# Sachin-A/TraceWeaver

Hardware: AMD Instinct MI355X
Metric: spans/sec reconstructed + assignment accuracy vs ground truth (higher is better)
Workload: dtype int64 timestamps, f64 scores; 1 GPU; media_microservices shape (6 services, E in {1,1,1,1,2,4}), 100000 requests/service x 16 replicas per GPU, concurrency 1.6, two-pass reconstruction, device mixture refit; spans_per_gpu=25600000, spans_total=25600000, parallelism=units sharded, 1 rank(s), backend none

## Files before the change

traceweaver_amd/csrc/tw_device.h:

```cpp
#pragma once
#include <hip/hip_runtime.h>
#include <stdint.h>

#include "traceweaver_amd.h"

namespace tw {

constexpr int kMaxEp = TW_MAX_EP;
constexpr int kTopK = TW_TOPK;
constexpr int kMaxComp = TW_MAX_COMP;
constexpr int kMaxWin = TW_MAX_WINDOW;
constexpr int kCandWords = TW_CAND_WORDS;
constexpr int kEnumStretches = 8;
constexpr int kTile = 128;
constexpr int kCoop = 256;
constexpr int32_t kNoOwner = 0x7f7f7f7f;

struct UnitDev {
    int64_t in_off;
    int64_t ie_off;
    int64_t ep_off[kMaxEp + 1];
    int32_t n_in;
    int32_t E;
    int32_t nblk;
// ... 31 lines not shown

struct Dev {
    const UnitDev* units;
    const TileDev* tiles;
    int32_t n_units, n_tiles;
    int32_t tile_spans;
    int64_t n_in_total, n_out_total;
    int32_t batch_size, batch_mis;
    const int64_t *in_start, *in_end, *out_start, *out_end;
    int64_t *in_end_sorted, *out_end_sorted;
    double* gparam;
    const int32_t* mix_n;
    const double* mix_c;
    int64_t* pm_val;
    int32_t* pm_idx;
    uint8_t* pc;
    int32_t* seg;
    uint8_t* win_end;
    int32_t* wid;
    int32_t* w_last;
    int32_t* unit_nwin;
    uint8_t* w_dirty;
    int32_t* w_conf;
    int32_t* unit_ndirty;
    int32_t* tk_n;
    int64_t* leaves;
    int64_t* leaves0;
    int32_t* chosen;
    uint8_t* rep;
    int32_t* tkr_n;
    int32_t *tk_idx, *tkr_idx;
    double *tk_score, *tkr_score;
    int32_t* c_lo;
    int32_t* c_hi;
    uint64_t* c_bits;
    uint64_t* gone;
    uint8_t* gone_valid;
    int64_t* leaves_r;
    unsigned long long* frontier_big;
    int32_t* frontier_big_busy;
    int32_t frontier_big_slots;
    int32_t* frontier_busy;
    unsigned long long* frontier;
    int32_t* round_changed;
    int32_t* parent;
    int32_t* owner;
    double* gaps;
    const int64_t* gs_off;
    int64_t* unit_stats;
    int32_t* heavy_count;
    int32_t* heavy_next;
    int32_t *heavy_unit, *heavy_win;
    int32_t *tiny_unit, *tiny_win;
    int32_t *rheavy_unit, *rheavy_win, *rtiny_unit, *rtiny_win;
    int32_t *hard_unit, *hard_win;
    int32_t* heavy_in_count;
    int32_t* heavy_in_next;
    int32_t heavy_in_off[kMaxEp + 2];
    int32_t* enum_snap;
    int32_t* enum_stretch_next;
    int32_t *heavy_in_unit, *heavy_in_idx;
    int32_t* heavy_big_count;
    int32_t *heavy_big_unit, *heavy_big_idx;
    int32_t heavy_big_off[kMaxEp + 2];
    int32_t* heavy_big_part;
    int32_t* heavy_big_slot;
    int32_t part_off[kMaxEp + 2];
    int32_t split_twins;
    int32_t* part_used;
    int32_t defer_min_e;
    int32_t defer_cap;
    unsigned long long* defer_list;
    int32_t* defer_used;
    int32_t* defer_count;
    int32_t *part_lo, *part_hi;
    int32_t* part_lvl;
    int32_t* any_wide;
    int32_t* redo_count;
    int32_t* defer_refused;
    int32_t lean_min_e;
    int32_t tile_max_deep;
    int32_t lean_grid;
    int32_t tile_rank;
    double* pair_pool;
    int32_t* pair_busy;
    int32_t* fb_count;
    int32_t* fb_total;
    int32_t *fb_unit, *fb_idx, *fb_part, *fb_slot;
    int32_t* split_count;
    int32_t *split_unit, *split_idx, *split_slot, *split_parts;
    int32_t* part_n;
    int64_t* part_leaves;
    double* part_score;
    int32_t* part_idx;
    unsigned long long* part_bits;
    int32_t* part_logn;
    double* part_log_sc;
    unsigned long long* part_log_ix;
    int32_t* err;
    unsigned long long* prof;
};

__device__ __forceinline__ int32_t hi_word(double x) { return (int32_t)(__double_as_longlong(x) >> 32); }
__device__ __forceinline__ uint32_t lo_word(double x) { return (uint32_t)__double_as_longlong(x); }
__device__ __forceinline__ double with_hi(double x, int32_t hi) {
    return __longlong_as_double((long long)(((uint64_t)(uint32_t)hi << 32) | (uint64_t)lo_word(x)));
}
__device__ __forceinline__ double dnan() { return __longlong_as_double(0x7ff8000000000000LL); }
__device__ __forceinline__ double dinf() { return __longlong_as_double(0x7ff0000000000000LL); }

__device__ inline double tw_log(double x) {
    const double ln2_hi = 6.93147180369123816490e-01, ln2_lo = 1.90821492927058770002e-10,
                 two54 = 1.80143985094819840000e+16, Lg1 = 6.666666666666735130e-01,
                 Lg2 = 3.999999999940941908e-01, Lg3 = 2.857142874366239149e-01,
                 Lg4 = 2.222219843214978396e-01, Lg5 = 1.818357216161805012e-01,
                 Lg6 = 1.531383769920937332e-01, Lg7 = 1.479819860511658591e-01;
    int32_t k = 0, hx = hi_word(x);
    if (hx < 0x00100000) {
        if (((hx & 0x7fffffff) | lo_word(x)) == 0) return -dinf();
        if (hx < 0) return dnan();
        k -= 54;
        x *= two54;
        hx = hi_word(x);
    }
    if (hx >= 0x7ff00000) return x + x;
    k += (hx >> 20) - 1023;
    hx &= 0x000fffff;
    int32_t i = (hx + 0x95f64) & 0x100000;
    x = with_hi(x, hx | (i ^ 0x3ff00000));
    k += (i >> 20);
    double f = x - 1.0, dk = (double)k;
    if ((0x000fffff & (2 + hx)) < 3) {
        if (f == 0.0) return k == 0 ? 0.0 : dk * ln2_hi + dk * ln2_lo;
        double R = f * f * (0.5 - 0.33333333333333333 * f);
        return k == 0 ? f - R : dk * ln2_hi - ((R - dk * ln2_lo) - f);
    }
    double s = f / (2.0 + f), z = s * s, w = z * z;
    i = hx - 0x6147a;
    int32_t j = 0x6b851 - hx;
    double t1 = w * (Lg2 + w * (Lg4 + w * Lg6));
    double t2 = z * (Lg1 + w * (Lg3 + w * (Lg5 + w * Lg7)));
    double R = t2 + t1;
    if ((i | j) > 0) {
        double hfsq = 0.5 * f * f;
        return k == 0 ? f - (hfsq - s * (hfsq + R)) : dk * ln2_hi - ((hfsq - (s * (hfsq + R) + dk * ln2_lo)) - f);
    }
    return k == 0 ? f - s * (f - R) : dk * ln2_hi - ((s * (f - R) - dk * ln2_lo) - f);
}

__device__ inline double tw_exp(double x) {
    const double o_threshold = 7.09782712893383973096e+02, u_threshold = -7.45133219101941108420e+02,
                 ln2HI = 6.93147180369123816490e-01, ln2LO = 1.90821492927058770002e-10,
                 invln2 = 1.44269504088896338700e+00, P1 = 1.66666666666666019037e-01,
                 P2 = -2.77777777770155933842e-03, P3 = 6.61375632143793436117e-05,
                 P4 = -1.65339022054652515390e-06, P5 = 4.13813679705723846039e-08,
                 twom1000 = 9.33263618503218878990e-302;
    double hi = 0.0, lo = 0.0;
    int32_t k = 0, hx = hi_word(x);
    const int32_t xsb = (hx >> 31) & 1;
    hx &= 0x7fffffff;
    if (hx >= 0x40862E42) {
        if (hx >= 0x7ff00000) {
            if (((hx & 0xfffff) | lo_word(x)) != 0) return x + x;
            return xsb == 0 ? x : 0.0;
        }
        if (x > o_threshold) return dinf();
// ... 139 lines not shown
```

traceweaver_amd/csrc/tw_engine.hip:

```cpp
#include <algorithm>
#include <chrono>
#include <cmath>
#include <cstdio>
#include <cstdlib>
#include <cstring>
#include <functional>
#include <string>
#include <type_traits>
#include <vector>

#include <hip/hip_runtime.h>
#include <rocprim/rocprim.hpp>

#include "traceweaver_amd.h"
#include "tw_kernels.h"
#include "tw_fit.h"
#include "tw_eval.h"
#include "tw_skip.h"
#include "tw_load.h"
#include "tw_baselines.h"
#include "tw_stitch.h"
#include "tw_attr.h"
#include "tw_conf.h"
#include "tw_dist.h"
#include "tw_sig.h"
#include "tw_prof.h"
#include "tw_order.h"

using namespace tw;

namespace {

constexpr int kMaxRepairRounds = 1 << 20;
enum { ST_EMPTY = 0, ST_LOADED = 1, ST_PASS1 = 2, ST_MIX = 3, ST_PASS2 = 4 };
enum { EV_BEGIN = 0, EV_PARAMS, EV_ENUM0, EV_ENUM1, EV_WIN, EV_SEL, EV_REPAIR, EV_END, EV_COUNT };
enum { SE_STITCH = 0, SE_ATTR = 5, SE_CONF = 9, SE_DIST = 13, SE_SIG = 18, SE_PROF = 22, SE_COUNT = 26 };

int env_int(const char* name, int dflt) {
    const char* v = getenv(name);
    return (v && *v) ? atoi(v) : dflt;
}

struct Mt19937 {
    uint32_t mt[624];
    int idx = 624;
    explicit Mt19937(uint32_t seed = 0u) {
        mt[0] = seed;
        for (int i = 1; i < 624; i++) mt[i] = 1812433253u * (mt[i - 1] ^ (mt[i - 1] >> 30)) + (uint32_t)i;
    }
    uint32_t next() {
        if (idx >= 624) {
            for (int i = 0; i < 624; i++) {
                const uint32_t y = (mt[i] & 0x80000000u) | (mt[(i + 1) % 624] & 0x7fffffffu);
                mt[i] = mt[(i + 397) % 624] ^ (y >> 1) ^ ((y & 1u) ? 0x9908b0dfu : 0u);
            }
            idx = 0;
        }
        uint32_t y = mt[idx++];
        y ^= y >> 11;
        y ^= (y << 7) & 0x9d2c5680u;
        y ^= (y << 15) & 0xefc60000u;
        y ^= y >> 18;
        return y;
    }
    double random_sample() {
        const uint32_t a = next() >> 5, b = next() >> 6;
        return ((double)a * 67108864.0 + (double)b) / 9007199254740992.0;
    }
};

}

struct tw_engine {
    int device = 0;
    hipStream_t stream = nullptr;
    hipStream_t cls_stream[kMaxEp + 1] = {};
    hipEvent_t cls_ev[kMaxEp + 2] = {};
    hipStream_t sel_stream[3] = {};
    hipStream_t sel_stream2[3] = {};
    int64_t select_fork_min = 0;
    hipEvent_t prep_ev = nullptr;
    hipEvent_t post_fork[kMaxEp + 1] = {}, post_join[kMaxEp + 1][3] = {}, post_done[kMaxEp + 1] = {};
    hipEvent_t tile_ev[kMaxEp + 1] = {};
    hipStream_t cls_stream2[kMaxEp + 1] = {};
    hipEvent_t stretch_ev[kMaxEp + 1][kEnumStretches] = {}, stretch_done[kMaxEp + 1] = {};
    int enum_stretches = 1, stretch_min_tiles = 2048;
    int heavy_grid = 4096, select_grid = 0;
    int debug_lists = 0;
    int32_t first_lists[3][kMaxEp + 1] = {};
    hipEvent_t gate_ev = nullptr;
    int tile_gate = 0;
    int stage_min_tiles = 1024;
    int32_t *rank_in = nullptr, *rank_out = nullptr;
    bool class_params = false;
    int prio_min_e = 0, prio_high = 0;
    bool prio_any = false;
    int pipeline = 1;
    std::string err;
    int state = ST_EMPTY;
    int tile = kTile;
    int tile_threads = 2;
    int tile_single = 1;
    int tile_rank = 1;
    int block_params = 1;
    int tile_single_threads = 1;
    int tile_pair = 1;
    int tile_pair_threads = 2;
    int coop = kCoop;
    std::vector<UnitDev> units;
    std::vector<TileDev> tiles;
    std::vector<int64_t> gs_off_h;
    std::vector<void*> allocs;
    void* arena = nullptr;
    size_t arena_cap = 0;
    bool arena_open = false;
    std::vector<std::pair<std::function<void(void*)>, size_t>> arena_req;
    Dev P{};
    int64_t n_ie = 0, n_gp = 0, n_slots = 0, n_gaps = 0;
    PairVI* agg_pair = nullptr;
    int32_t *agg_i32 = nullptr, *agg_i32b = nullptr;
    uint32_t *seg_in = nullptr, *seg_out = nullptr;
    int n_seg_out = 0;
    void* sort_tmp = nullptr;
    size_t sort_tmp_bytes = 0;
    double* mix_p_dev = nullptr;
    int32_t* mix_n_dev = nullptr;
    double* mix_c_dev = nullptr;
    double* gaps_sorted = nullptr;
    double* fit_models = nullptr;
    double* fit_uval = nullptr;
    int32_t *fit_ustart = nullptr, *fit_row_n = nullptr, *fit_row_uniq = nullptr;
    double* fit_centres = nullptr;
    double *fit_tape = nullptr, *fit_tape100 = nullptr;
    int64_t* fit_tape_off = nullptr;
    int64_t fit_tape_cap = 0;
    bool fit_runs_pending = false;
    bool fit_prepared = false;
    int tile_sub_max = 8;
    int32_t hard_pass1[kMaxEp + 1] = {};
    int8_t wide_pass1[kMaxEp + 1] = {};
    int32_t split_pass1[kMaxEp + 1] = {};
    int lean_pool = 512;
    bool pass1_done = false;
    std::vector<int32_t> fit_max_n;
    bool fit_max_n_valid = false;
    Mt19937 fit_rng;
    uint32_t fit_seed = 0;
    int32_t* slot_unit = nullptr;
    int32_t* tile_ids = nullptr;
    int32_t* ctr = nullptr;
    int64_t ctr_round_ints = 0, ctr_pass_ints = 0;
    int32_t tile_cls_off[kMaxEp + 2] = {};
    BlockRef* blk_tab = nullptr;
    int32_t blk_cls_off[kMaxEp + 2] = {};
    uint32_t *seg_gap = nullptr, *seg_gap_end = nullptr, *seg_gap_dst = nullptr;
    unsigned long long *comp_a = nullptr, *comp_b = nullptr;
    int64_t comp_cap = 0, n_gap_scored = 0;
    int32_t *truth = nullptr, *in_trace = nullptr;
    uint8_t* trace_bad = nullptr;
    unsigned long long* eval_counts = nullptr;
    int64_t n_traces = 0, trace_cap = 0;
    uint8_t* slot_scored = nullptr;
    int64_t n_gap_rows = 0;
    unsigned long long* key_acc = nullptr;
    double fit_ms = 0.0;
    int rounds = 0;
    bool skip_mode = false;
    SkipUnitDev* skip_units = nullptr;
    int32_t* skip_perm = nullptr; int64_t* skip_tw = nullptr; int32_t* skip_pool = nullptr; double* skip_dist = nullptr; long long* skip_fetch = nullptr;
    int64_t skip_fetch_n = 0;
    int64_t *orig_is = nullptr, *orig_ie = nullptr, *orig_os = nullptr, *orig_oe = nullptr;
    int32_t *orig_truth = nullptr, *orig_trace = nullptr;
    bool scaled_upload = false;
    hipEvent_t ev[EV_COUNT] = {};
    double ms[6] = {0, 0, 0, 0, 0, 0};
    StitchDev S{};
    int32_t* given_parent = nullptr;
    bool rows_set = false, parents_given = false, stitched = false;
    int64_t rows_cap = 0, st_trees = 0;
    int stitched_pass = -1;
    bool stitched_truth = false;
    AttrDev A{};
    bool groups_set = false, attributed = false;
    int64_t groups_cap = 0, attr_rows_cap = 0;
    ConfDev C{};
    int64_t conf_rows_cap = 0;
// ... 694 lines not shown
    int32_t* d_rank = trace_rank != nullptr ? (int32_t*)scratch(4 * n_in) : nullptr;
    unsigned long long *ka = (unsigned long long*)scratch(8 * n_max), *kb = (unsigned long long*)scratch(8 * n_max);
    uint32_t *perm = (uint32_t*)scratch(4 * n_max), *perm_alt = (uint32_t*)scratch(4 * n_max);
    uint32_t* perm_in = (uint32_t*)scratch(4 * n_in);
    int32_t *pos_in = (int32_t*)scratch(4 * n_in), *pos_out = (int32_t*)scratch(4 * n_out);
    if (!L.x || !L.xe || !L.y || !L.ye || !L.rank_in || !L.rank_out || !L.row_in || !L.row_out || !L.owner_req || !L.kmax || !L.err || !d_factor ||
        !d_segbase || (trace_rank != nullptr && !d_rank) || !ka || !kb || !perm || !perm_alt || !perm_in || !pos_in || !pos_out)
        return fail(e, TW_ERR_DEVICE, "tw_scale_load: out of device memory");
    std::vector<int32_t> segbase_h((size_t)P.n_units);
    { int32_t acc = 0; for (int u = 0; u < P.n_units; u++) { segbase_h[(size_t)u] = acc; acc += e->units[(size_t)u].E; } }
    HIPCHK(hipMemcpyAsync(d_factor, unit_factor, sizeof(int32_t) * P.n_units, hipMemcpyHostToDevice, e->stream));
    HIPCHK(hipMemcpyAsync(d_segbase, segbase_h.data(), sizeof(int32_t) * P.n_units, hipMemcpyHostToDevice, e->stream));
    if (d_rank != nullptr) HIPCHK(hipMemcpyAsync(d_rank, trace_rank, sizeof(int32_t) * n_in, hipMemcpyHostToDevice, e->stream));
    L.factor = d_factor; L.seg_base = d_segbase; L.trace_rank = d_rank;
    HIPCHK(hipMemsetAsync(L.kmax, 0, sizeof(int32_t) * P.n_units, e->stream));
    HIPCHK(hipMemsetAsync(L.err, 0, sizeof(int32_t), e->stream));
    HIPCHK(hipMemsetAsync(L.owner_req, 0xff, sizeof(int32_t) * n_out, e->stream));
    hipLaunchKernelGGL(k_load_scale_in, dim3(P.n_tiles), dim3(e->tile), 0, e->stream, L);
    hipLaunchKernelGGL(k_load_scale_out, dim3(P.n_tiles), dim3(e->tile), 0, e->stream, L);
    hipLaunchKernelGGL(k_load_to_int, dim3(P.n_tiles), dim3(e->tile), 0, e->stream, L);
    HIPCHK(hipGetLastError());
    std::vector<int32_t> kmax_h((size_t)P.n_units);
    int32_t err_h = 0;
    HIPCHK(hipMemcpyAsync(kmax_h.data(), L.kmax, sizeof(int32_t) * P.n_units, hipMemcpyDeviceToHost, e->stream));
    HIPCHK(hipMemcpyAsync(&err_h, L.err, sizeof(int32_t), hipMemcpyDeviceToHost, e->stream));
    HIPCHK(hipStreamSynchronize(e->stream));
    if (err_h != 0)
        return fail(e, TW_ERR_ARG, "tw_scale_load: the requests' own calls are not one call per request at every endpoint (helpers/transforms.py:25-29 asserts it), "
                                   "or the scaled timestamps span too many binades for int64");
    const unsigned grid_in = (unsigned)std::min<int64_t>((n_in + 255) / 256, 8192), grid_out = (unsigned)std::min<int64_t>((n_out + 255) / 256, 8192);
    const unsigned block = flat_threads(e);
    int64_t* d_is = const_cast<int64_t*>(P.in_start); int64_t* d_ie = const_cast<int64_t*>(P.in_end);
    int64_t* d_os = const_cast<int64_t*>(P.out_start); int64_t* d_oe = const_cast<int64_t*>(P.out_end);
    for (int side = 0; side < 2; side++) {
        const int64_t n = side == 0 ? n_in : n_out;
        const int64_t* vs = (const int64_t*)(side == 0 ? L.x : L.y); const int64_t* ve = (const int64_t*)(side == 0 ? L.xe : L.ye);
        const int32_t* rank = side == 0 ? L.rank_in : L.rank_out; const int32_t* row = side == 0 ? L.row_in : L.row_out;
        const int nrows = side == 0 ? P.n_units : e->n_seg_out;
        unsigned bs = 0, be = 0;
        rc = differing_bits(e, vs, n, &bs); if (rc != TW_OK) return rc;
        rc = differing_bits(e, ve, n, &be); if (rc != TW_OK) return rc;
        hipLaunchKernelGGL(k_load_iota, dim3(side == 0 ? grid_in : grid_out), dim3(block), 0, e->stream, perm, n);
        rc = load_sort_pass(e, rank, n, 32u, ka, kb, &perm, &perm_alt); if (rc != TW_OK) return rc;
        rc = load_sort_pass(e, ve, n, be, ka, kb, &perm, &perm_alt); if (rc != TW_OK) return rc;
        rc = load_sort_pass(e, vs, n, bs, ka, kb, &perm, &perm_alt); if (rc != TW_OK) return rc;
        rc = load_sort_pass(e, row, n, std::max(1u, bit_length((unsigned long long)std::max(nrows - 1, 1))), ka, kb, &perm, &perm_alt); if (rc != TW_OK) return rc;
        hipLaunchKernelGGL(k_load_place, dim3(side == 0 ? grid_in : grid_out), dim3(block), 0, e->stream, (const uint32_t*)perm, n, vs, ve,
                           side == 0 ? d_is : d_os, side == 0 ? d_ie : d_oe, side == 0 ? pos_in : pos_out);
        hipLaunchKernelGGL(k_load_local, dim3(side == 0 ? grid_in : grid_out), dim3(block), 0, e->stream, perm, row, (const uint32_t*)(side == 0 ? e->seg_in : e->seg_out), n);
        HIPCHK(hipGetLastError());
        int32_t* host = side == 0 ? in_perm : out_perm;
        if (host != nullptr) HIPCHK(hipMemcpyAsync(host, perm, sizeof(uint32_t) * n, hipMemcpyDeviceToHost, e->stream));
        HIPCHK(hipStreamSynchronize(e->stream));
    }
    hipLaunchKernelGGL(k_load_retruth, dim3(P.n_tiles), dim3(e->tile), 0, e->stream, L, (const int32_t*)pos_in, (const int32_t*)pos_out, e->truth,
                       has_trace ? e->in_trace : nullptr);
    HIPCHK(hipGetLastError());
    for (int u = 0; u < P.n_units; u++) {
        UnitDev& U = e->units[(size_t)u];
        U.tscale = std::ldexp(1.0, -kmax_h[(size_t)u]);
        U.float_time = 1;
        if (unit_time_scale != nullptr) unit_time_scale[u] = U.tscale;
    }
    HIPCHK(hipMemcpyAsync(const_cast<UnitDev*>(P.units), e->units.data(), sizeof(UnitDev) * e->units.size(), hipMemcpyHostToDevice, e->stream));
    HIPCHK(hipStreamSynchronize(e->stream));
    e->state = ST_LOADED; e->pass1_done = false;
    drop_batch_order(e);
    for (int E = 0; E <= kMaxEp; E++) { e->wide_pass1[E] = -1; e->hard_pass1[E] = -1; e->split_pass1[E] = -1; }
    return TW_OK;
}

extern "C" {

int tw_create(int device_id, tw_engine** out) {
    if (out == nullptr) return TW_ERR_ARG;
    *out = nullptr;
    tw_engine* e = new tw_engine();
    e->device = device_id;
    e->tile = std::min(std::max(env_int("TW_TILE", kTile), 1), kTile);
    e->tile_threads = std::min(std::max(env_int("TW_TILE_THREADS", 2), 1), 4);
    e->tile_single = env_int("TW_TILE_SINGLE", 1);
    e->block_params = env_int("TW_BLOCK_PARAMS", 1);
    e->tile_rank = env_int("TW_TILE_RANK", 1) != 0 ? 1 : 0;
    e->tile_single_threads = std::min(std::max(env_int("TW_TILE_SINGLE_THREADS", 1), 1), 4);
    e->tile_pair = env_int("TW_TILE_PAIR", 1);
    e->tile_pair_threads = std::min(std::max(env_int("TW_TILE_PAIR_THREADS", 2), 1), 2);
    e->coop = std::min(std::max(env_int("TW_COOP_THREADS", kCoop), 1), kCoop);
    if (env_int("TW_SET_HW_QUEUES", 0) != 0) setenv("GPU_MAX_HW_QUEUES", "12", 0);
    hipError_t s = hipSetDevice(device_id);
    if (s == hipSuccess) s = hipStreamCreate(&e->stream);
    for (int i = 0; i < EV_COUNT && s == hipSuccess; i++) s = hipEventCreate(&e->ev[i]);
    for (int i = 0; i < SE_COUNT && s == hipSuccess; i++) s = hipEventCreate(&e->stage_ev[i]);
    const int prio_min_e = env_int("TW_PRIO_MIN_E", 0);
    int prio_least = 0, prio_greatest = 0;
    if (s == hipSuccess) s = hipDeviceGetStreamPriorityRange(&prio_least, &prio_greatest);
    e->prio_min_e = prio_min_e; e->prio_high = prio_greatest; e->prio_any = prio_greatest != prio_least;
    for (int i = 0; i <= kMaxEp + 1 && s == hipSuccess; i++) s = hipEventCreateWithFlags(&e->cls_ev[i], hipEventDisableTiming);
    if (s == hipSuccess) s = hipEventCreateWithFlags(&e->prep_ev, hipEventDisableTiming);
    for (int i = 0; i <= kMaxEp && s == hipSuccess; i++) {
        s = hipEventCreateWithFlags(&e->post_fork[i], hipEventDisableTiming);
        if (s == hipSuccess) s = hipEventCreateWithFlags(&e->tile_ev[i], hipEventDisableTiming);
        if (s == hipSuccess) s = hipEventCreateWithFlags(&e->post_done[i], hipEventDisableTiming);
        if (s == hipSuccess) s = hipEventCreateWithFlags(&e->stretch_done[i], hipEventDisableTiming);
        for (int j = 0; j < kEnumStretches && s == hipSuccess; j++) s = hipEventCreateWithFlags(&e->stretch_ev[i][j], hipEventDisableTiming);
        for (int j = 0; j < 3 && s == hipSuccess; j++) s = hipEventCreateWithFlags(&e->post_join[i][j], hipEventDisableTiming);
    }
    e->pipeline = env_int("TW_CLASS_PIPELINE", 1);
    e->sig_hash_bits = std::min(std::max(env_int("TW_SIG_HASH_BITS", 64), 1), 64);
    e->tile_gate = env_int("TW_TILE_GATE", 0);
    e->enum_stretches = std::min(std::max(env_int("TW_ENUM_STRETCHES", 1), 1), kEnumStretches);
    e->heavy_grid = std::max(env_int("TW_HEAVY_GRID", 4096), 64);
    e->select_grid = std::max(env_int("TW_SELECT_GRID", 0), 0);
    e->debug_lists = env_int("TW_DEBUG_LISTS", 0);
    e->select_fork_min = (int64_t)env_int("TW_SELECT_FORK_MIN", 0);
    e->stretch_min_tiles = std::max(env_int("TW_STRETCH_MIN_TILES", 2048), 1);
    e->stage_min_tiles = env_int("TW_STAGE_MIN_TILES", 1024);
    e->tile_sub_max = std::max(env_int("TW_TILE_SUB", 8), 1);
    e->lean_pool = std::min(std::max(env_int("TW_LEAN_POOL", 512), 1), 4096);
    if (s != hipSuccess) {
        fprintf(stderr, "tw_create: %s\n", hipGetErrorString(s));
        delete e;
        return TW_ERR_DEVICE;
    }
    *out = e;
    return TW_OK;
}

void tw_destroy(tw_engine* e) {
    if (e == nullptr) return;
    (void)hipSetDevice(e->device);
    free_all(e);
    order_unstage(e);
    if (e->arena != nullptr) (void)hipFree(e->arena);
    for (int i = 0; i < EV_COUNT; i++)
        if (e->ev[i]) (void)hipEventDestroy(e->ev[i]);
    for (int i = 0; i <= kMaxEp + 1; i++)
        if (e->cls_ev[i]) (void)hipEventDestroy(e->cls_ev[i]);
    for (int i = 1; i <= kMaxEp; i++)
        if (e->cls_stream[i]) (void)hipStreamDestroy(e->cls_stream[i]);
    for (int i = 0; i < 3; i++) {
        if (e->sel_stream[i]) (void)hipStreamDestroy(e->sel_stream[i]);
        if (e->sel_stream2[i]) (void)hipStreamDestroy(e->sel_stream2[i]);
    }
    if (e->prep_ev) (void)hipEventDestroy(e->prep_ev);
    for (int i = 0; i <= kMaxEp; i++) {
        if (e->post_fork[i]) (void)hipEventDestroy(e->post_fork[i]);
        if (e->tile_ev[i]) (void)hipEventDestroy(e->tile_ev[i]);
        if (e->post_done[i]) (void)hipEventDestroy(e->post_done[i]);
        if (e->stretch_done[i]) (void)hipEventDestroy(e->stretch_done[i]);
        for (int j = 0; j < kEnumStretches; j++)
            if (e->stretch_ev[i][j]) (void)hipEventDestroy(e->stretch_ev[i][j]);
        if (e->cls_stream2[i]) (void)hipStreamDestroy(e->cls_stream2[i]);
        for (int j = 0; j < 3; j++)
            if (e->post_join[i][j]) (void)hipEventDestroy(e->post_join[i][j]);
    }
    for (int i = 0; i < SE_COUNT; i++)
        if (e->stage_ev[i]) (void)hipEventDestroy(e->stage_ev[i]);
    if (e->stream) (void)hipStreamDestroy(e->stream);
    delete e;
}

const char* tw_last_error(const tw_engine* e) { return e ? e->err.c_str() : "null engine"; }

int tw_load_batch(tw_engine* e, const tw_batch* b, int spans_on_device) {
    if (e == nullptr || b == nullptr) return TW_ERR_ARG;
    HIPCHK(hipSetDevice(e->device));
// ... 92 lines not shown
    int32_t heavy_off_h[kMaxEp + 2] = {};
    for (int cls = 0; cls <= kMaxEp; cls++) {
        e->tile_cls_off[cls] = (int32_t)tile_ids_h.size();
        heavy_off_h[cls + 1] = heavy_off_h[cls];
        for (size_t tix = 0; tix < e->tiles.size(); tix++)
            if (e->units[(size_t)e->tiles[tix].unit].E == cls) tile_ids_h.push_back((int32_t)tix);
        for (int u = 0; u < b->n_units; u++)
            if (e->units[(size_t)u].E == cls) heavy_off_h[cls + 1] += e->units[(size_t)u].n_in;
    }
    e->tile_cls_off[kMaxEp + 1] = (int32_t)tile_ids_h.size();
    std::vector<BlockRef> blk_tab_h;
    for (int cls = 0; cls <= kMaxEp; cls++) {
        e->blk_cls_off[cls] = (int32_t)blk_tab_h.size();
        for (int u = 0; u < b->n_units; u++)
            if (cls == 0 || e->units[(size_t)u].E == cls)
                for (int k = 0; k < e->units[(size_t)u].nblk; k += param_group(e->units[(size_t)u].E)) blk_tab_h.push_back(BlockRef{u, k});
    }
    e->blk_cls_off[kMaxEp + 1] = (int32_t)blk_tab_h.size();
    for (int cls = 1; cls <= kMaxEp; cls++)
        if (e->tile_cls_off[cls + 1] > e->tile_cls_off[cls]) {
            int rs = ensure_class_stream(e, cls); if (rs != TW_OK) return rs;
            if (e->enum_stretches > 1 && e->tile_cls_off[cls + 1] - e->tile_cls_off[cls] >= 2 * e->stretch_min_tiles && e->cls_stream2[cls] == nullptr)
                HIPCHK(hipStreamCreate(&e->cls_stream2[cls]));
        }
    for (int j = 0; j < 3; j++)
        if (e->sel_stream[j] == nullptr) HIPCHK(hipStreamCreate(&e->sel_stream[j]));
    {
        bool want = false;
        int deepest = 0;
        for (int cls = 1; cls <= kMaxEp; cls++) if (e->tile_cls_off[cls + 1] > e->tile_cls_off[cls]) deepest = cls;
        for (int cls = 1; cls < deepest; cls++) want |= e->select_fork_min > 0 && heavy_off_h[cls + 1] - heavy_off_h[cls] >= e->select_fork_min;
        for (int j = 0; j < 3 && want; j++)
            if (e->sel_stream2[j] == nullptr) HIPCHK(hipStreamCreate(&e->sel_stream2[j]));
    }
    const int64_t n_in_total = b->unit_in_off[b->n_units], n_out_total = b->ep_off[epi];
    if (n_in_total >= (1ll << 31) || n_out_total >= (1ll << 31)) return fail(e, TW_ERR_ARG, "batch exceeds 2^31 spans");
    if (gaps >= (1ll << 31)) return fail(e, TW_ERR_ARG, "batch too large: sum of nslot*n_in must stay below 2^31");
    std::vector<int32_t> slot_unit_h;
    std::vector<uint8_t> slot_scored_h;
    std::vector<uint32_t> seg_gap_h, seg_gap_end_h;
    for (int u = 0; u < b->n_units; u++) {
        const UnitDev& U = e->units[(size_t)u];
        const int E = U.E;
        for (int q = 0; q < U.nslot; q++) {
            bool scored;
            if (q < E) scored = U.npred[q] == 0;
            else if (q < E + E * E) {
                const int p = (q - E) / E, en = (q - E) % E;
                scored = false;
                for (int j = 0; j < U.npred[en]; j++) scored |= (U.pred_list[en][j] == p && U.pred_prim[en][j]);
            } else scored = true;
            slot_unit_h.push_back(u);
            slot_scored_h.push_back(scored ? 1 : 0);
            if (scored) {
                seg_gap_h.push_back((uint32_t)(e->gs_off_h[(size_t)u] + (int64_t)q * U.n_in));
                seg_gap_end_h.push_back((uint32_t)(e->gs_off_h[(size_t)u] + (int64_t)(q + 1) * U.n_in));
            }
        }
    }
    e->n_gap_rows = (int64_t)seg_gap_h.size();
    std::vector<uint32_t> seg_gap_dst_h(seg_gap_h.size());
    e->n_gap_scored = 0;
    for (size_t r = 0; r < seg_gap_h.size(); r++) { seg_gap_dst_h[r] = (uint32_t)e->n_gap_scored; e->n_gap_scored += seg_gap_end_h[r] - seg_gap_h[r]; }
    seg_in[(size_t)b->n_units] = (uint32_t)n_in_total;
    seg_out.push_back((uint32_t)n_out_total);
    e->n_seg_out = (int)seg_out.size() - 1;
    e->n_ie = ie; e->n_gp = gp; e->n_slots = slots; e->n_gaps = gaps;

    Dev& P = e->P;
    P = Dev{};
    P.n_units = b->n_units;
    P.n_tiles = (int32_t)e->tiles.size();
    P.tile_spans = e->tile;
    P.n_in_total = n_in_total;
    P.n_out_total = n_out_total;
    P.batch_size = b->batch_size;
    P.batch_mis = b->batch_size_mis;
    P.split_twins = env_int("TW_SPLIT_TWINS", 2);
    P.defer_min_e = env_int("TW_DEFER_MIN_E", 5);
    P.lean_min_e = env_int("TW_LEAN_MIN_E", 5);
    P.lean_grid = std::max(env_int("TW_LEAN_GRID", TW_LEAN_GRID), 1);
    P.tile_max_deep = std::min(std::max(env_int("TW_TILE_MAX_DEEP", kTileMax), 0), kTileMax);
    P.tile_rank = e->tile_rank;
    int rc;
    e->arena_req.clear();
    e->arena_open = true;
    UnitDev* d_units; TileDev* d_tiles; int64_t *d_is, *d_ie, *d_os, *d_oe, *d_gs;
    DEV_ALLOC(d_units, P.n_units); DEV_ALLOC(d_tiles, P.n_tiles);
    DEV_ALLOC(d_is, n_in_total); DEV_ALLOC(d_ie, n_in_total); DEV_ALLOC(d_os, n_out_total); DEV_ALLOC(d_oe, n_out_total);
    DEV_ALLOC(d_gs, P.n_units);
    DEV_ALLOC(P.in_end_sorted, n_in_total); DEV_ALLOC(P.out_end_sorted, n_out_total);
    DEV_ALLOC(P.gparam, gp * 4);
    DEV_ALLOC(e->mix_n_dev, slots); DEV_ALLOC(e->mix_p_dev, slots * kMaxComp * 3); DEV_ALLOC(e->mix_c_dev, slots * kMaxComp * 4);
    DEV_ALLOC(P.pm_val, n_in_total); DEV_ALLOC(P.pm_idx, n_in_total); DEV_ALLOC(P.pc, n_in_total + 1); DEV_ALLOC(P.seg, n_in_total);
    DEV_ALLOC(P.win_end, n_in_total); DEV_ALLOC(P.wid, n_in_total); DEV_ALLOC(P.w_last, n_in_total);
    DEV_ALLOC(P.unit_nwin, P.n_units); DEV_ALLOC(P.w_dirty, n_in_total); DEV_ALLOC(P.w_conf, n_in_total);
    DEV_ALLOC(P.tk_n, n_in_total); DEV_ALLOC(P.leaves, n_in_total); DEV_ALLOC(P.leaves0, n_in_total); DEV_ALLOC(P.chosen, n_in_total); DEV_ALLOC(P.rep, n_in_total);
    DEV_ALLOC(P.tkr_n, n_in_total);
    DEV_ALLOC(P.tk_idx, ie * kTopK); DEV_ALLOC(P.tkr_idx, ie * kTopK);
    DEV_ALLOC(P.tk_score, n_in_total * kTopK); DEV_ALLOC(P.tkr_score, n_in_total * kTopK);
    DEV_ALLOC(P.c_lo, ie); DEV_ALLOC(P.c_hi, ie); DEV_ALLOC(P.c_bits, ie * kCandWords); DEV_ALLOC(P.parent, ie);
    DEV_ALLOC(P.gone, ie * kCandWords); DEV_ALLOC(P.gone_valid, n_in_total); DEV_ALLOC(P.leaves_r, n_in_total);
    DEV_ALLOC(P.frontier, (int64_t)kFrontierSlots * 2 * kFrontierCap); 
    P.frontier_big_slots = (int32_t)std::min<int64_t>(std::max<int64_t>(n_in_total / 16384, kFrontierBigSlots), std::max(kFrontierBigSlots, 512));
    DEV_ALLOC(P.frontier_big, (int64_t)P.frontier_big_slots * 2 * kFrontierBigCap);
    DEV_ALLOC(P.pair_pool, (int64_t)kPairSlots * kPairSpill);
    DEV_ALLOC(P.owner, n_out_total);
    DEV_ALLOC(P.gaps, gaps);
    DEV_ALLOC(e->tile_ids, (int64_t)tile_ids_h.size());
    DEV_ALLOC(e->blk_tab, (int64_t)blk_tab_h.size());
    DEV_ALLOC(P.heavy_in_unit, n_in_total); DEV_ALLOC(P.heavy_in_idx, n_in_total);
    {
        int64_t big_total = 0, slots = 0, want = 0;
        for (int cls = 0; cls <= kMaxEp; cls++) want += 2 * part_extra(cls, heavy_off_h[cls + 1] - heavy_off_h[cls]);
        static const int64_t slots_max = (int64_t)std::max(env_int("TW_PART_SLOTS_MAX", 16 << 20), 1024);
        for (int cls = 0; cls <= kMaxEp; cls++) {
            const int64_t n_cls = heavy_off_h[cls + 1] - heavy_off_h[cls];
            int64_t extra = part_extra(cls, n_cls);
            if (want > slots_max && extra > 64) extra = std::max<int64_t>((int64_t)((double)extra * (double)slots_max / (double)want), std::min<int64_t>(n_cls / 8 + 64, extra));
            P.heavy_big_off[cls] = (int32_t)big_total; P.part_off[cls] = (int32_t)slots;
            big_total += n_cls + extra; slots += 2 * extra;
        }
        P.heavy_big_off[kMaxEp + 1] = (int32_t)big_total; P.part_off[kMaxEp + 1] = (int32_t)slots;
        DEV_ALLOC(P.heavy_big_unit, big_total); DEV_ALLOC(P.heavy_big_idx, big_total);
        DEV_ALLOC(P.heavy_big_part, big_total); DEV_ALLOC(P.heavy_big_slot, big_total);
        DEV_ALLOC(P.fb_unit, big_total); DEV_ALLOC(P.fb_idx, big_total); DEV_ALLOC(P.fb_part, big_total); DEV_ALLOC(P.fb_slot, big_total);
        DEV_ALLOC(P.split_unit, slots); DEV_ALLOC(P.split_idx, slots); DEV_ALLOC(P.split_slot, slots); DEV_ALLOC(P.split_parts, slots);
        DEV_ALLOC(P.part_n, slots); DEV_ALLOC(P.part_leaves, slots); DEV_ALLOC(P.part_score, slots * kTopK); DEV_ALLOC(P.part_idx, slots * kTopK * kMaxEp);
        DEV_ALLOC(P.part_bits, slots * kMaxEp * kCandWords);
        DEV_ALLOC(P.part_logn, slots); DEV_ALLOC(P.part_log_sc, slots * kPartLogCap); DEV_ALLOC(P.part_log_ix, slots * kPartLogCap);
        DEV_ALLOC(P.part_lo, slots); DEV_ALLOC(P.part_hi, slots); DEV_ALLOC(P.part_lvl, slots);
        int64_t deep = 0;
        for (int cls = std::max(P.defer_min_e, 3); cls <= kMaxEp; cls++) deep += heavy_off_h[cls + 1] - heavy_off_h[cls];
        P.defer_cap = (int32_t)(deep > 0 ? std::min<int64_t>(std::max<int64_t>(deep * kDeferListPerSpan, kDeferListMin), 1ll << 28) : 1);
        DEV_ALLOC(P.defer_list, P.defer_cap);
    }
    for (int cls = 0; cls <= kMaxEp + 1; cls++) P.heavy_in_off[cls] = heavy_off_h[cls];
    DEV_ALLOC(P.prof, 32); DEV_ALLOC(e->key_acc, 2);
    const int64_t sel_cap = (int64_t)P.n_tiles * e->tile + 1;
    {
        int64_t at = 0;
        auto take = [&](int64_t ints) { const int64_t o = at; at += (ints + 31) / 32 * 32; return o; };
        const int64_t o_hc = take(kSelSlots * 4 * kSelSeg * kCtrStride), o_hn = take(kSelSlots * 8), o_ic = take(2 * (kMaxEp + 1)), o_in = take(8 * (kMaxEp + 1)), o_bc = take(kMaxEp + 1),
                      o_rc = take(1), o_rd = take(kMaxEp + 1), o_fc = take(kMaxEp + 1);
        e->ctr_round_ints = at;
        const int64_t o_pu = take(kMaxEp + 1), o_sc = take(kMaxEp + 1), o_dc = take(kMaxEp + 1), o_du = take(1), o_err = take(1), o_nd = take(P.n_units), o_us = take((int64_t)P.n_units * 16);
        const int64_t o_dr = take(kMaxEp + 1), o_ft = take(kMaxEp + 1), o_aw = take(kMaxEp + 1);
        const int64_t o_es = take((kMaxEp + 1) * (kEnumStretches + 1) * 4), o_en = take((kMaxEp + 1) * kEnumStretches * 2);
        const int64_t o_fn = take(kFrontierSlots), o_fb = take(P.frontier_big_slots), o_pb = take(kPairSlots);
        e->ctr_pass_ints = at;
        auto place = [=](void* q) {
            Dev& D = e->P;
            int32_t* c = e->ctr = (int32_t*)q;
            D.heavy_count = c + o_hc; D.heavy_next = c + o_hn; D.heavy_in_count = c + o_ic; D.heavy_in_next = c + o_in; D.heavy_big_count = c + o_bc;
            D.round_changed = c + o_rc; D.frontier_busy = c + o_fn; D.frontier_big_busy = c + o_fb;
            D.defer_count = c + o_dc; D.defer_used = c + o_du;
            D.part_used = c + o_pu; D.split_count = c + o_sc; D.err = c + o_err; D.unit_ndirty = c + o_nd;
            D.redo_count = c + o_rd; D.fb_count = c + o_fc; D.defer_refused = c + o_dr; D.fb_total = c + o_ft; D.pair_busy = c + o_pb; D.any_wide = c + o_aw;
            D.enum_snap = c + o_es; D.enum_stretch_next = c + o_en;
            D.unit_stats = (int64_t*)(c + o_us);
        };
        if (e->arena_open) e->arena_req.emplace_back(place, ((size_t)at * sizeof(int32_t) + 255) / 256 * 256);
        else { DEV_ALLOC(e->ctr, at); place(e->ctr); }
    }
    DEV_ALLOC(P.heavy_unit, sel_cap); DEV_ALLOC(P.heavy_win, sel_cap);
    DEV_ALLOC(P.tiny_unit, sel_cap); DEV_ALLOC(P.tiny_win, sel_cap);
// ... 1752 lines not shown
```

traceweaver_amd/csrc/tw_tile.h:

```cpp
#pragma once

namespace tw {

#ifndef TW_TILE_MAX
#define TW_TILE_MAX 256
#endif
constexpr int kTileMax = TW_TILE_MAX;
#ifndef TW_TILE_REPLAY_MAX
#define TW_TILE_REPLAY_MAX 256
#endif
constexpr int kTileReplayMax = TW_TILE_REPLAY_MAX;
#ifndef TW_TILE_RANK_DIRECT
#define TW_TILE_RANK_DIRECT 32
#endif
constexpr int kRankDirect = TW_TILE_RANK_DIRECT;
constexpr int kRankMinLong = (kRankDirect & ~3) + 4;
constexpr int kRankBuckets = 5;
static_assert(kRankDirect >= 24, "the maxima and counters of a segment's long spans lie in one byte per tuple slot");
__device__ __forceinline__ uint32_t score_key32(double v) {
    const unsigned long long u = (unsigned long long)__double_as_longlong(v + 0.0);
    return (uint32_t)(((u >> 63) ? ~u : (u | (1ull << 63))) >> 32);
}
__device__ __forceinline__ int pos_base(unsigned long long pk, int e) {
    int acc = 0;
// ... 131 lines not shown
        return term_gauss(g[0], g[3], g[2], x);
    }
    return score_term_mix_x(S, slot, x);
}

#ifdef TW_PROFILE_TILE
#ifndef TW_PROFILE_TILE_E
#define TW_PROFILE_TILE_E 4
#endif
#define TW_TILE_T0() long long _tp = wall_clock64(); const long long _tb = _tp; long long _ta[7] = {0, 0, 0, 0, 0, 0, 0}
#define TW_TILE_TICK(k) do { const long long _n = wall_clock64(); _ta[k] += _n - _tp; _tp = _n; } while (0)
#define TW_TILE_COUNT(k, v) do { if (E == TW_PROFILE_TILE_E && threadIdx.x == 0) atomicAdd((unsigned long long*)&P.prof[k], (unsigned long long)(v)); } while (0)
#define TW_TILE_FLUSH() do { if (E == TW_PROFILE_TILE_E && threadIdx.x == 0) { for (int _k = 0; _k < 7; _k++) atomicAdd((unsigned long long*)&P.prof[_k], (unsigned long long)_ta[_k]); \
    atomicAdd((unsigned long long*)&P.prof[7], (unsigned long long)(wall_clock64() - _tb)); atomicAdd((unsigned long long*)&P.prof[8], 1ull); } } while (0)
#else
#define TW_TILE_T0() do {} while (0)
#define TW_TILE_TICK(k) do {} while (0)
#define TW_TILE_COUNT(k, v) do {} while (0)
#define TW_TILE_FLUSH() do {} while (0)
#endif

#ifdef TW_HOST_EMULATION
#define TW_TILE_ATTR
#else
#ifndef TW_TILE_PAIR_WAVES
#define TW_TILE_PAIR_WAVES 4
#endif
#define TW_TILE_ATTR __attribute__((amdgpu_waves_per_eu(SINGLE ? 8 : (PAIR ? TW_TILE_PAIR_WAVES : (E <= 4 ? 4 : 2)))))
#endif
template <int E, int SPANS = kTile, bool SINGLE = false, bool PAIR = false>
__global__ void __launch_bounds__(4 * kTile) TW_TILE_ATTR k_enumerate_tile(Dev P, int pass, const int32_t* tile_ids, int n_tiles_e, int sub_tiles) {
    static_assert(!SINGLE || E == 1, "the lean path is the one of a single endpoint");
    static_assert(!PAIR || (E == 2 && !SINGLE), "the pair path is the one of two endpoints");
    if (*P.err != 0) return;
    typedef TileCfg<E, SPANS, PAIR> C;
    constexpr int SL = C::kSlice;
    const int vb = xcd_tile(blockIdx.x, n_tiles_e * sub_tiles);
    const int tile = tile_ids[vb / sub_tiles];
    const TileDev T = P.tiles[tile];
    const UnitDev& U = P.units[T.unit];
    const int t = threadIdx.x, nt = blockDim.x;
    const int sub_spans = P.tile_spans / sub_tiles, first = T.first + (vb % sub_tiles) * sub_spans;
    const int ns = min(sub_spans, min(P.tile_spans, U.n_in - T.first) - (vb % sub_tiles) * sub_spans);
    if (ns <= 0) return;
    __shared__ int32_t s_is[SPANS], s_ie[SPANS];
    __shared__ int32_t sl_st[E][SL], sl_en[E][SL];
    __shared__ int32_t s_A[E], s_B[E];
    __shared__ uint16_t s_lo[E][SPANS];
    __shared__ uint32_t s_cm[E][SPANS];
    __shared__ uint32_t s_bits[E][SPANS];
    __shared__ int32_t s_item0[SPANS + 1], s_grid0[SPANS + 1], s_leaves[SPANS];
    __shared__ uint8_t s_amb[SPANS];
    __shared__ unsigned long long s_cn[SPANS];
    __shared__ int32_t s_wtot[4 * kTile / 64][2];
    __shared__ double t_root[C::kItems], t_close[C::kItems];
    __shared__ uint16_t it_idx[C::kItems];
    __shared__ double g_sc[C::kGrid + (PAIR ? 4 : 0)];
    __shared__ uint8_t g_span[C::kGrid];
    __shared__ uint32_t g_aux[C::kGrid / 4];
    __shared__ int32_t s_segend, s_anyamb;
    const bool live = t < ns;
    const int i = first + (live ? t : 0);
    const int64_t base = P.in_start[U.in_off + first];
    const int64_t in_start = P.in_start[U.in_off + i], in_end = P.in_end[U.in_off + i];
    const int64_t* os[E];
    const int64_t* oe[E];
#pragma unroll
    for (int e = 0; e < E; e++) { os[e] = P.out_start + U.ep_off[e]; oe[e] = P.out_end + U.ep_off[e]; }
    for (int x = t; x < E; x += nt) { s_A[x] = 0x7fffffff; s_B[x] = 0; }
    uint32_t dag_pm[E], dag_np[E], dag_pl[E];
    uint32_t ordered = 0;
#pragma unroll
    for (int e = 0; e < E; e++) {
        dag_pm[e] = U.pred_mask[e];
        dag_np[e] = U.npred[e];
        uint32_t pk = 0;
#pragma unroll
        for (int j = 0; j < E; j++) pk |= (j < (int)dag_np[e] ? ((uint32_t)U.pred_list[e][j] | ((uint32_t)U.pred_prim[e][j] << 3)) : 0u) << (4 * j);
        dag_pl[e] = pk;
        ordered |= dag_pm[e];
    }
    TW_TILE_T0();
    int32_t lo[E], hi[E];
    if ((t & ~63) >= ns) {
#pragma unroll
        for (int e = 0; e < E; e++) { lo[e] = 0; hi[e] = -1; }
    } else if (pass == 1) {
#pragma unroll
        for (int e = E - 1; e >= 0; e--) {
            const int n = (int)(U.ep_off[e + 1] - U.ep_off[e]);
            int64_t tmax = in_end;
#pragma unroll
            for (int f = e + 1; f < E; f++) {
                if (!((U.succ_mask[e] >> f) & 1)) continue;
                const int nf = (int)(U.ep_off[f + 1] - U.ep_off[f]);
                const int anchor = hi[f] >= 0 ? hi[f] : nf - 1;
                const int64_t st = os[f][anchor];
                if (st < tmax) tmax = st;
            }
            if (U.skip) {
                lo[e] = lower_bound_i64(os[e], n, in_start);
                hi[e] = upper_bound_i64(os[e], n, tmax) - 1;
            } else {
                lo[e] = bound_near<false>(os[e], n, in_start, i);
                hi[e] = bound_near<true>(os[e], n, tmax, lo[e]) - 1;
            }
        }
        if (live) {
#pragma unroll
            for (int e = 0; e < E; e++) { P.c_lo[ie_index(U, e, i)] = lo[e]; P.c_hi[ie_index(U, e, i)] = hi[e]; }
        }
    } else {
#pragma unroll
        for (int e = 0; e < E; e++) { lo[e] = P.c_lo[ie_index(U, e, i)]; hi[e] = P.c_hi[ie_index(U, e, i)]; }
    }
    bool wide = false, empty = false, narrow = true;
#pragma unroll
    for (int e = 0; e < E; e++) {
        const int w = hi[e] - lo[e] + 1;
        wide |= (w > 64 * kCandWords);
        narrow &= (w <= kNarrow);
        empty |= (w <= 0);
    }
    if (live && wide) { raise_err(P, TW_ERR_WINDOW_WIDTH); }
    group_sync();
    TW_TILE_TICK(0);
    {
        const bool in = live && !empty && !wide;
#pragma unroll
        for (int e = 0; e < E; e++) {
            int a = in ? lo[e] : 0x7fffffff, b = in ? hi[e] + 1 : 0;
            for (int off = 32; off >= 1; off >>= 1) { const int a2 = __shfl_xor(a, off), b2 = __shfl_xor(b, off); a = a2 < a ? a2 : a; b = b2 > b ? b2 : b; }
            if ((t & 63) == 0) { atomicMin(&s_A[e], a); atomicMax(&s_B[e], b); }
        }
    }
    group_sync();
    int32_t cnt[E];
#pragma unroll
    for (int e = 0; e < E; e++) { const int c = s_B[e] - s_A[e]; cnt[e] = c < 0 ? 0 : (c > SL ? SL : c); }
    if (E >= P.lean_min_e && P.tile_max_deep == 0) {
#pragma unroll
        for (int e = 0; e < E; e++) cnt[e] = 0;
    }
    auto clamp32 = [](long long v) -> int32_t { return (int32_t)(v > 0x7fffffffll ? 0x7fffffffll : (v < -0x7fffffffll ? -0x7fffffffll : v)); };
    for (int x0 = 0; x0 < SL; x0 += nt) {
        const int x = x0 + t;
        int64_t a[E], b[E];
#pragma unroll
        for (int e = 0; e < E; e++) { a[e] = 0; b[e] = 0; if (x < cnt[e]) { a[e] = os[e][s_A[e] + x]; b[e] = oe[e][s_A[e] + x]; } }
#pragma unroll
        for (int e = 0; e < E; e++) if (x < cnt[e]) { sl_st[e][x] = clamp32(a[e] - base); sl_en[e][x] = clamp32(b[e] - base); }
    }
    group_sync();
    TW_TILE_TICK(1);
    const long long iso = in_start - base, ieo = in_end - base;
    const bool far = iso < 0 || ieo >= 0x7fffffffll || in_end < in_start || in_end - in_start >= (1ll << 31);
    uint32_t cm[E];
    bool fits = narrow && !far && !empty;
    long long prod = empty ? 0 : 1;
#pragma unroll
    for (int e = 0; e < E; e++) {
        cm[e] = 0;
        const int rel = lo[e] - s_A[e], w = hi[e] - lo[e] + 1;
        if (fits && (rel < 0 || rel + w > cnt[e])) fits = false;
        if (fits) {
            for (int r = 0; r < w; r++)
                if (sl_st[e][rel + r] >= (int32_t)iso && sl_en[e][rel + r] <= (int32_t)ieo) cm[e] |= 1u << r;
            prod = prod <= kTileMax ? prod * __popcll((unsigned long long)cm[e]) : prod;
        }
    }
    const long long tile_max = E >= P.lean_min_e ? (long long)P.tile_max_deep : (long long)kTileMax;
    const bool mine = live && !wide && (empty || (fits && prod <= tile_max));
    {
        long long hprod = 0;
        int first_cands = 0;
        bool twins_any = false;
        if (live && !mine && !wide) {
            hprod = 1;
            bool twins = false;
#pragma unroll
            for (int e = 0; e < E; e++) {
                int v = 0;
                const int rel = lo[e] - s_A[e], w = hi[e] - lo[e] + 1;
                if (!far && rel >= 0 && rel + w <= cnt[e]) {
                    int32_t prev = -0x7fffffff - 1;
                    for (int r = 0; r < w; r++) {
                        const int32_t st = sl_st[e][rel + r];
                        if (st >= (int32_t)iso && sl_en[e][rel + r] <= (int32_t)ieo) { v++; twins |= st == prev; prev = st; }
                    }
                } else {
                    int64_t prev = INT64_MIN;
                    for (int cx = lo[e]; cx <= hi[e]; cx++) {
                        const int64_t st = os[e][cx];
                        if (st >= in_start && oe[e][cx] <= in_end) { v++; twins |= st == prev; prev = st; }
                    }
                }
                if (hprod <= (1ll << 40)) hprod *= v;
                if (e == 0) first_cands = v;
            }
            if (twins && P.split_twins == 0) first_cands = 0;
            twins_any = twins;
            if (E >= P.lean_min_e) first_cands = 0;
            if (E >= 3 && E >= P.defer_min_e) {
                uint32_t any_order = 0;
#pragma unroll
                for (int e = 0; e < E; e++) any_order |= U.pred_mask[e];
                if (any_order != 0) first_cands = 0;
            }
        }
        heavy_append<E>(P, live && !mine && !wide, narrow, hprod > kBigProduct, T.unit, i, hprod, U.skip ? 0 : first_cands, twins_any);
    }
    const bool some = mine && !empty && prod > 0;
    int nitem = 0;
    unsigned long long cnpack = 0;
    if (live) {
#pragma unroll
        for (int e = 0; e < E; e++) {
            const int rel = lo[e] - s_A[e], c = some ? __popcll((unsigned long long)cm[e]) : 0;
            s_lo[e][t] = (uint16_t)(some ? rel : 0);
            s_cm[e][t] = some ? cm[e] : 0u;
            if constexpr (!SINGLE) s_bits[e][t] = 0u;
            nitem += c;
            cnpack |= (unsigned long long)c << (8 * e);
        }
        s_is[t] = (int32_t)iso; s_ie[t] = (int32_t)ieo;
        s_amb[t] = 0;
        if constexpr (!SINGLE) { s_cn[t] = cnpack; s_leaves[t] = (some && !ordered) ? (int)prod : 0; }
    }
    {
        int a = live ? nitem : 0, b = (!SINGLE && live && some) ? (PAIR ? (int)prod : (((int)prod + 3) & ~3)) : 0;
        const int lane = t & 63, wv = t >> 6;
        for (int off = 1; off < 64; off <<= 1) {
            const int a2 = __shfl_up(a, off);
            if (lane >= off) a += a2;
            if constexpr (!SINGLE) { const int b2 = __shfl_up(b, off); if (lane >= off) b += b2; }
        }
        if (lane == 63 || t == nt - 1) { s_wtot[wv][0] = a; if constexpr (!SINGLE) s_wtot[wv][1] = b; }
        group_sync();
        for (int w = 0; w < wv; w++) { a += s_wtot[w][0]; if constexpr (!SINGLE) b += s_wtot[w][1]; }
// ... 564 lines not shown
```

Measured before the change: 1.382 billion spans/s.

## Stage tile-wide outgoing window in LDS and compute pass-1 cutoffs from it

In pass 1 the tile first finds a shared outgoing-span window per endpoint with a coalesced probe, stages it into LDS, and then derives each span's lo/hi bounds by binary search over the staged int32 offsets instead of per-thread global bound searches. The later slice load reuses the staged data, shifting it in place when the window start differs, and falls back to the old path when the window does not fit. This aims to cut scattered global memory reads in the bounds phase, at the cost of extra probing, synchronisation and more complex code.

```diff
diff --git a/traceweaver_amd/csrc/tw_device.h b/traceweaver_amd/csrc/tw_device.h
--- a/traceweaver_amd/csrc/tw_device.h
+++ b/traceweaver_amd/csrc/tw_device.h
@@ -137,6 +137,7 @@
     int32_t tile_max_deep;
     int32_t lean_grid;
     int32_t tile_rank;
+    int32_t tile_cutoffs;
     double* pair_pool;
     int32_t* pair_busy;
     int32_t* fb_count;
diff --git a/traceweaver_amd/csrc/tw_engine.hip b/traceweaver_amd/csrc/tw_engine.hip
--- a/traceweaver_amd/csrc/tw_engine.hip
+++ b/traceweaver_amd/csrc/tw_engine.hip
@@ -102,6 +102,7 @@
     int tile_threads = 2;
     int tile_single = 1;
     int tile_rank = 1;
+    int tile_cutoffs = 1;
     int block_params = 1;
     int tile_single_threads = 1;
     int tile_pair = 1;
@@ -962,6 +963,7 @@
     e->tile_single = env_int("TW_TILE_SINGLE", 1);
     e->block_params = env_int("TW_BLOCK_PARAMS", 1);
     e->tile_rank = env_int("TW_TILE_RANK", 1) != 0 ? 1 : 0;
+    e->tile_cutoffs = env_int("TW_TILE_CUTOFFS", 1) != 0 ? 1 : 0;
     e->tile_single_threads = std::min(std::max(env_int("TW_TILE_SINGLE_THREADS", 1), 1), 4);
     e->tile_pair = env_int("TW_TILE_PAIR", 1);
     e->tile_pair_threads = std::min(std::max(env_int("TW_TILE_PAIR_THREADS", 2), 1), 2);
@@ -1220,6 +1222,7 @@
     P.lean_grid = std::max(env_int("TW_LEAN_GRID", TW_LEAN_GRID), 1);
     P.tile_max_deep = std::min(std::max(env_int("TW_TILE_MAX_DEEP", kTileMax), 0), kTileMax);
     P.tile_rank = e->tile_rank;
+    P.tile_cutoffs = e->tile_cutoffs;
     int rc;
     e->arena_req.clear();
     e->arena_open = true;
diff --git a/traceweaver_amd/csrc/tw_tile.h b/traceweaver_amd/csrc/tw_tile.h
--- a/traceweaver_amd/csrc/tw_tile.h
+++ b/traceweaver_amd/csrc/tw_tile.h
@@ -237,28 +237,126 @@
     }
     TW_TILE_T0();
     int32_t lo[E], hi[E];
+    const long long iso = in_start - base, ieo = in_end - base;
+    const bool far = iso < 0 || ieo >= 0x7fffffffll || in_end < in_start || in_end - in_start >= (1ll << 31);
+    auto clamp32 = [](long long v) -> int32_t { return (int32_t)(v > 0x7fffffffll ? 0x7fffffffll : (v < -0x7fffffffll ? -0x7fffffffll : v)); };
+    static_assert(2 * E <= SPANS + 1, "the tile's bounds of every endpoint lie in s_item0");
+    bool staged = false;
+    if (pass == 1 && P.tile_cutoffs != 0 && !U.skip && !(E >= P.lean_min_e && P.tile_max_deep == 0)) {
+        int32_t tend = (live && !far) ? (int32_t)ieo : 0;
+        for (int off = 32; off >= 1; off >>= 1) { const int32_t t2 = __shfl_xor(tend, off); tend = t2 > tend ? t2 : tend; }
+        if ((t & 63) == 0) s_wtot[t >> 6][0] = tend;
+        for (int q = t; q < 2 * E; q += nt) s_item0[q] = 0x7fffffff;
+        group_sync();
+        int32_t tmo = 0;
+        for (int w = 0; w < (nt + 63) / 64; w++) tmo = s_wtot[w][0] > tmo ? s_wtot[w][0] : tmo;
+        constexpr int kProbe = 32, kNone = 0x7fffffff;
+        auto probe0 = [&](int up, int n) -> int {
+            const int w0 = up ? first + ns - kProbe / 4 : first - 3 * kProbe / 4;
+            return w0 < 0 ? 0 : (w0 > n ? n : w0);
+        };
+        const bool grouped = nt == 1 || (nt & 63) == 0;
+        if (grouped) {
+            for (int x0 = 0; x0 < 2 * E * kProbe; x0 += nt) {
+                const int idx = x0 + t, q = idx / kProbe, e = q >> 1, up = q & 1;
+                int32_t found = kNone;
+                if (idx < 2 * E * kProbe) {
+                    const int64_t* a = P.out_start + U.ep_off[e];
+                    const int n = (int)(U.ep_off[e + 1] - U.ep_off[e]);
+                    const int pos = probe0(up, n) + idx % kProbe;
+                    if (pos < n) {
+                        const int64_t v = a[pos];
+                        if (up ? v > base + tmo : v >= base) found = pos;
+                    }
+                }
+                for (int off = kProbe / 2; off >= 1; off >>= 1) { const int32_t f2 = __shfl_xor(found, off); found = f2 < found ? f2 : found; }
+                if (idx < 2 * E * kProbe && (nt == 1 || idx % kProbe == 0) && found != kNone) atomicMin(&s_item0[up * E + e], found);
+            }
+            group_sync();
+        }
+        for (int q = t; q < 2 * E; q += nt) {
+            const int e = q >> 1, up = q & 1;
+            const int64_t* a = P.out_start + U.ep_off[e];
+            const int n = (int)(U.ep_off[e + 1] - U.ep_off[e]);
+            const int w0 = probe0(up, n), w1 = w0 + kProbe < n ? w0 + kProbe : n;
+            int r = s_item0[up * E + e];
+            bool ok = grouped;
+            if (r == kNone) { r = w1; ok = ok && w1 == n; }
+            ok = ok && (r > w0 || w0 == 0);
+            if (!ok) r = up ? bound_near<true>(a, n, base + tmo, first + ns) : bound_near<false>(a, n, base, first);
+            s_item0[up * E + e] = r;
+        }
+        group_sync();
+        staged = true;
+#pragma unroll
+        for (int e = 0; e < E; e++) staged &= s_item0[E + e] - s_item0[e] <= SL;
+        if (staged) {
+            for (int x0 = 0; x0 < SL; x0 += nt) {
+                const int x = x0 + t;
+                int64_t a[E], b[E];
+#pragma unroll
+                for (int e = 0; e < E; e++) { a[e] = 0; b[e] = 0; if (x < s_item0[E + e] - s_item0[e]) { a[e] = os[e][s_item0[e] + x]; b[e] = oe[e][s_item0[e] + x]; } }
+#pragma unroll
+                for (int e = 0; e < E; e++) if (x < s_item0[E + e] - s_item0[e]) { sl_st[e][x] = clamp32(a[e] - base); sl_en[e][x] = clamp32(b[e] - base); }
+            }
+            group_sync();
+        }
+    }
     if ((t & ~63) >= ns) {
 #pragma unroll
         for (int e = 0; e < E; e++) { lo[e] = 0; hi[e] = -1; }
     } else if (pass == 1) {
-#pragma unroll
-        for (int e = E - 1; e >= 0; e--) {
-            const int n = (int)(U.ep_off[e + 1] - U.ep_off[e]);
-            int64_t tmax = in_end;
-#pragma unroll
-            for (int f = e + 1; f < E; f++) {
-                if (!((U.succ_mask[e] >> f) & 1)) continue;
-                const int nf = (int)(U.ep_off[f + 1] - U.ep_off[f]);
-                const int anchor = hi[f] >= 0 ? hi[f] : nf - 1;
-                const int64_t st = os[f][anchor];
-                if (st < tmax) tmax = st;
-            }
-            if (U.skip) {
-                lo[e] = lower_bound_i64(os[e], n, in_start);
-                hi[e] = upper_bound_i64(os[e], n, tmax) - 1;
-            } else {
-                lo[e] = bound_near<false>(os[e], n, in_start, i);
-                hi[e] = bound_near<true>(os[e], n, tmax, lo[e]) - 1;
+        bool done = staged && !far;
+        if (done) {
+            constexpr int kTop = SL >= 128 ? 128 : (SL >= 64 ? 64 : (SL >= 32 ? 32 : 16));
+            static_assert(SL >= kTop && 2 * kTop > SL, "the steps reach every count up to SL");
+            auto count_before = [&](const int32_t* sl, int c, int32_t v, bool with) -> int {
+                int pos = 0;
+#pragma unroll
+                for (int step = kTop; step >= 1; step >>= 1) {
+                    const int np = pos + step;
+                    const int32_t x = sl[(np <= SL ? np : SL) - 1];
+                    if (np <= c && (with ? x <= v : x < v)) pos = np;
+                }
+                return pos;
+            };
+#pragma unroll
+            for (int e = 0; e < E; e++) lo[e] = s_item0[e] + count_before(sl_st[e], s_item0[E + e] - s_item0[e], (int32_t)iso, false);
+#pragma unroll
+            for (int e = E - 1; e >= 0; e--) {
+                const int tA = s_item0[e], c = s_item0[E + e] - tA;
+                int32_t tmo = (int32_t)ieo;
+#pragma unroll
+                for (int f = e + 1; f < E; f++) {
+                    if (!((U.succ_mask[e] >> f) & 1)) continue;
+                    int rel = hi[f] - s_item0[f];
+                    if (rel < 0 || rel >= s_item0[E + f] - s_item0[f]) { done = false; rel = 0; }
+                    const int32_t st = sl_st[f][rel];
+                    if (st < tmo) tmo = st;
+                }
+                hi[e] = tA + count_before(sl_st[e], c, tmo, true) - 1;
+            }
+        }
+        if (!done) {
+#pragma unroll
+            for (int e = E - 1; e >= 0; e--) {
+                const int n = (int)(U.ep_off[e + 1] - U.ep_off[e]);
+                int64_t tmax = in_end;
+#pragma unroll
+                for (int f = e + 1; f < E; f++) {
+                    if (!((U.succ_mask[e] >> f) & 1)) continue;
+                    const int nf = (int)(U.ep_off[f + 1] - U.ep_off[f]);
+                    const int anchor = hi[f] >= 0 ? hi[f] : nf - 1;
+                    const int64_t st = os[f][anchor];
+                    if (st < tmax) tmax = st;
+                }
+                if (U.skip) {
+                    lo[e] = lower_bound_i64(os[e], n, in_start);
+                    hi[e] = upper_bound_i64(os[e], n, tmax) - 1;
+                } else {
+                    lo[e] = bound_near<false>(os[e], n, in_start, i);
+                    hi[e] = bound_near<true>(os[e], n, tmax, lo[e]) - 1;
+                }
             }
         }
         if (live) {
@@ -297,19 +395,37 @@
 #pragma unroll
         for (int e = 0; e < E; e++) cnt[e] = 0;
     }
-    auto clamp32 = [](long long v) -> int32_t { return (int32_t)(v > 0x7fffffffll ? 0x7fffffffll : (v < -0x7fffffffll ? -0x7fffffffll : v)); };
-    for (int x0 = 0; x0 < SL; x0 += nt) {
-        const int x = x0 + t;
-        int64_t a[E], b[E];
-#pragma unroll
-        for (int e = 0; e < E; e++) { a[e] = 0; b[e] = 0; if (x < cnt[e]) { a[e] = os[e][s_A[e] + x]; b[e] = oe[e][s_A[e] + x]; } }
-#pragma unroll
-        for (int e = 0; e < E; e++) if (x < cnt[e]) { sl_st[e][x] = clamp32(a[e] - base); sl_en[e][x] = clamp32(b[e] - base); }
+    bool shift = false;
+    if (staged) {
+#pragma unroll
+        for (int e = 0; e < E; e++) {
+            const int d = s_A[e] - s_item0[e];
+            if (cnt[e] > 0 && (d < 0 || d + cnt[e] > s_item0[E + e] - s_item0[e])) staged = false;
+            shift |= cnt[e] > 0 && d > 0;
+        }
+    }
+    if (!staged) {
+        for (int x0 = 0; x0 < SL; x0 += nt) {
+            const int x = x0 + t;
+            int64_t a[E], b[E];
+#pragma unroll
+            for (int e = 0; e < E; e++) { a[e] = 0; b[e] = 0; if (x < cnt[e]) { a[e] = os[e][s_A[e] + x]; b[e] = oe[e][s_A[e] + x]; } }
+#pragma unroll
+            for (int e = 0; e < E; e++) if (x < cnt[e]) { sl_st[e][x] = clamp32(a[e] - base); sl_en[e][x] = clamp32(b[e] - base); }
+        }
+    } else if (shift) {
+        for (int x0 = 0; x0 < SL; x0 += nt) {
+            const int x = x0 + t;
+            int32_t a[E], b[E];
+#pragma unroll
+            for (int e = 0; e < E; e++) { const int d = s_A[e] - s_item0[e]; a[e] = 0; b[e] = 0; if (x < cnt[e] && d > 0) { a[e] = sl_st[e][x + d]; b[e] = sl_en[e][x + d]; } }
+            group_sync();
+#pragma unroll
+            for (int e = 0; e < E; e++) { const int d = s_A[e] - s_item0[e]; if (x < cnt[e] && d > 0) { sl_st[e][x] = a[e]; sl_en[e][x] = b[e]; } }
+        }
     }
     group_sync();
     TW_TILE_TICK(1);
-    const long long iso = in_start - base, ieo = in_end - base;
-    const bool far = iso < 0 || ieo >= 0x7fffffffll || in_end < in_start || in_end - in_start >= (1ll << 31);
     uint32_t cm[E];
     bool fits = narrow && !far && !empty;
     long long prod = empty ? 0 : 1;
```

Result: no change. 1.388 billion spans/s, median of 6 (+0.4%).
